# lxjeffffff/PagedAttention-Based-Transformer-Decoder-Inference-Framework

Hardware: AMD Instinct MI355X
Metric: decode tokens/sec at batch=64 seq_len=8192; % HBM-roofline (1/2/4/8 GPU) (higher is better)
Workload: dtype int8 GEMM (i32 acc) + fp16 KV attention (fp32 acc); 1 GPU; C3: INT8 decoder (MFMA i8 matmuls + fp16 paged attention), 24-layer/16-head/d=128, batch 64, KV context 8192, page 16; strong scaling: 64 rows over 1 GPU(s); global_batch=64, batch_per_gpu=64, seq_len=8192, page_size=16, parallelism=single GPU (no collective)

## Files before the change

### pagedattention-based-transformer-decoder-inference-framework_amd/csrc/gemm_impl.hpp

```cpp
#pragma once

#include "common.hpp"
#include "fp8.hpp"
#include "gemm.hpp"
#include "ln_wave.hpp"

namespace llm {

struct KvAppend {
  const int32_t* pos;
  const int32_t* page_table;
  const int32_t* rows;
  _Float16* k_pool;
  _Float16* v_pool;
  int num_beams, max_tiles, TS, num_pages, H, D;
  size_t page_stride;
  int fp8;
  float k_inv, v_inv;
};

struct GemmArgs {
  const uint8_t* A;
  int lda;
  int a_packed;
  const uint8_t* B;
  int M, N, K, KS;
  const float* sa;
  const float* sw;
  const float* bias;
  int act;
  float* C;
  int32_t* acc_out;
  int c_cols;
  int c_ld;
  _Float16* c16;
  KvAppend kv;
  unsigned long long* stamps;
  const float* ln_x;
  const _Float16* ln_emb;
  const int32_t* ln_tok;
  int ln_V;
  const float* ln_g;
  const float* ln_b;
  float ln_eps;
  uint8_t* act_out;
  float* sa_out;
  int partial;
  int w_keep;
  int xcd_map;
  unsigned* seam;
  int seam_n;
  int qdiag;
  int ksplit2;
};

__host__ __device__ constexpr int ln_row_stride(int K, int esize) { return K * esize + 32; }

__device__ __forceinline__ unsigned long long phase_clock() {
  unsigned long long t;
  asm volatile("s_memrealtime %0\n\ts_waitcnt lgkmcnt(0)" : "=s"(t)::"memory");
  return t;
}


template <int MT, int WAVES, int NT = 1>
constexpr int gemm_unroll() {
  return (MT >= 4 ? 2 : 4) * (WAVES == 4 ? 2 : 1) / (NT >= 4 ? 2 : 1);
}

__device__ __forceinline__ float apply_act(float y, int act) {
  if (act == LLM_ACT_RELU) return fmaxf(y, 0.f);
  if (act == LLM_ACT_GELU) return 0.5f * y * (1.f + erff(y * 0.70710678118654752f));
  return y;
}

enum class GemmKind { I8, F16 };

template <GemmKind KIND>
struct GemmTraits;
template <>
struct GemmTraits<GemmKind::I8> {
  static constexpr int KSTEP = 64, ESIZE = 1;
  using acc_t = i32x4;
  using elem_t = int32_t;
};
template <>
struct GemmTraits<GemmKind::F16> {
  static constexpr int KSTEP = 32, ESIZE = 2;
  using acc_t = f32x4;
  using elem_t = float;
};

template <GemmKind KIND, int ROWS, int WAVES>
__device__ __forceinline__ void ln_prologue(const GemmArgs& a, int m0, uint8_t* alds,
                                            float* sa_lds) {
  constexpr int ESIZE = GemmTraits<KIND>::ESIZE;
  constexpr int CPL = 8;
  const int lane = lane_id();
  const int w = wave_id_uniform();
  const int K = a.K;
  const int K4 = K >> 2;
  const int stride = ln_row_stride(K, ESIZE);
  const bool do_ln = a.ln_g != nullptr;
  LnRow<CPL> gm, bt;
  ln_wave_load(a.ln_g, K4, do_ln, gm);
  ln_wave_load(a.ln_b, K4, do_ln, bt);
  for (int r0 = w; r0 < ROWS; r0 += 2 * WAVES) {
    LnRow<CPL> x[2];
#pragma unroll
    for (int q = 0; q < 2; ++q) {
      const int r = r0 + q * WAVES;
      const int m = m0 + r;
      const bool ok = r < ROWS && m < a.M;
      if (a.ln_emb)
        ln_wave_load_f16(ok ? ln_embed_row(a.ln_emb, a.ln_tok, m, a.ln_V, K) : a.ln_emb, K4, ok,
                         x[q]);
      else
        ln_wave_load(a.ln_x + (size_t)m * K, K4, ok, x[q]);
    }
#pragma unroll
    for (int q = 0; q < 2; ++q) {
      const int r = r0 + q * WAVES;
      if (r >= ROWS) break;
      const bool mok = m0 + r < a.M;
      float am;
      if (do_ln) {
        am = ln_wave_compute(x[q], gm, bt, K, a.ln_eps);
      } else {
        am = 0.f;
#pragma unroll
        for (int j = 0; j < CPL; ++j)
#pragma unroll
          for (int e = 0; e < 4; ++e) am = fmaxf(am, fabsf(x[q].v[j][e]));
        am = ln_wave_max(am);
      }
      uint8_t* rowp = alds + (size_t)r * stride;
      if constexpr (KIND == GemmKind::I8) {
        const float scale = 127.f / (am + 1e-6f);
#pragma unroll
        for (int j = 0; j < CPL; ++j) {
          const int c = 64 * j + lane;
          if (c < K4)
            *reinterpret_cast<uint32_t*>(rowp + 4 * c) = mok ? ln_quant4(x[q].v[j], scale) : 0u;
        }
        if (lane == 0) sa_lds[r] = mok ? 1.0f / scale : 0.f;
      } else {
#pragma unroll
        for (int j = 0; j < CPL; ++j) {
          const int c = 64 * j + lane;
          if (c < K4)
            *reinterpret_cast<ln_f16x4*>(rowp + 8 * c) =
                mok ? ln_half4(x[q].v[j]) : ln_f16x4{0, 0, 0, 0};
        }
      }
    }
  }
}

__device__ __forceinline__ void seam_wait(unsigned* ctr, int n) {
  if (threadIdx.x == 0) {
    unsigned spins = 0;
    while (__hip_atomic_load(&ctr[0], __ATOMIC_RELAXED, __HIP_MEMORY_SCOPE_AGENT) < (unsigned)n) {
      __builtin_amdgcn_s_sleep(8);
      if (++spins > (1u << 21)) {
        __hip_atomic_store(&ctr[2], 1u, __ATOMIC_RELAXED, __HIP_MEMORY_SCOPE_AGENT);
        break;
      }
    }
    __builtin_amdgcn_fence(__ATOMIC_ACQUIRE, "agent");
  }
  __syncthreads();
}

template <GemmKind KIND, int MT, int NT, int WAVES, int DIAG = 0, int PRO = 0, int SEAM = 0>
__device__ __forceinline__ void gemm_tile(const GemmArgs& a, int bx, int by, int bz, int nz,
                                          int gx) {
  using Tr = GemmTraits<KIND>;
  using acc_t = typename Tr::acc_t;
  constexpr int KSTEP = Tr::KSTEP;
  constexpr int kUnroll = gemm_unroll<MT, WAVES, NT>();
  using elem_t = typename Tr::elem_t;
  using RedT = elem_t[MT * NT][4][64];
  extern __shared__ __attribute__((aligned(16))) uint8_t gemm_smem[];
  RedT* red;
  if constexpr (PRO == 0) {
    __shared__ elem_t red_static[WAVES][MT * NT][4][64];
    red = red_static;
  } else {
    red = reinterpret_cast<RedT*>(gemm_smem);
  }
  constexpr int ROWS_ = 16 * MT;
  const int a_stride = ln_row_stride(a.K, Tr::ESIZE);
  uint8_t* alds = gemm_smem;
  float* sa_lds = reinterpret_cast<float*>(gemm_smem + (size_t)ROWS_ * a_stride);

  const int lane = lane_id();
  const int w = wave_id_uniform();
  const int nt0 = bx * NT;
  const int m0 = by * 16 * MT;
  unsigned long long* stamp =
      a.stamps ? a.stamps + ((size_t)by * gx + bx) * 48 : nullptr;
  if (stamp && lane == 0) stamp[w] = phase_clock();
  const int wr = (w + bx) % WAVES;
  const int kz0 = (int)((bz * a.KS) / nz);
  const int kzn = (int)(((bz + 1) * a.KS) / nz) - kz0;
  const int ks0 = kz0 + (wr * kzn) / WAVES;
  const int ks1 = kz0 + ((wr + 1) * kzn) / WAVES;
  const int ntiles = (a.N + 15) >> 4;

  const int arow_lane = lane & 15;
  const int kgrp = lane >> 4;
  const bool apk = a.a_packed;
  const uint32_t a_bytes = apk ? (uint32_t)(((a.M + 15) / 16) * a.KS * 1024u)
                               : (uint32_t)((size_t)a.M * a.lda * Tr::ESIZE);
  const auto arsrc = __builtin_amdgcn_make_buffer_rsrc((void*)a.A, (short)0, a_bytes, 0x00020000);
  const uint32_t a_kstride = apk ? 1024u : (uint32_t)(KSTEP * Tr::ESIZE);
  const uint32_t a_kgrp_off = apk ? 0u : (uint32_t)(kgrp * (KSTEP / 4) * Tr::ESIZE);
  uint32_t a_row_off[MT];
#pragma unroll
  for (int mt = 0; mt < MT; ++mt) {
    const int row = m0 + mt * 16 + arow_lane;
    a_row_off[mt] = row >= a.M ? 0xFFFFFFF0u
                    : apk ? (uint32_t)((((m0 >> 4) + mt) * a.KS) * 1024u + lane * 16)
                          : (uint32_t)((size_t)row * a.lda * Tr::ESIZE);
  }
  const uint8_t* bbase = a.B + (size_t)nt0 * a.KS * 1024;
  const uint32_t b_bytes = (uint32_t)(min(NT, ntiles - nt0) * a.KS * 1024u);
  uint32_t b_lane_off[NT];
#pragma unroll
  for (int j = 0; j < NT; ++j) b_lane_off[j] = (uint32_t)j * a.KS * 1024u + lane * 16;
  const auto brsrc = __builtin_amdgcn_make_buffer_rsrc((void*)bbase, (short)0, b_bytes, 0x00020000);

  acc_t acc[MT][NT];
#pragma unroll
  for (int mt = 0; mt < MT; ++mt)
#pragma unroll
    for (int j = 0; j < NT; ++j) acc[mt][j] = acc_t{0, 0, 0, 0};

  struct Batch {
    u32x4 b[kUnroll][NT];
    u32x4 af[kUnroll][MT];
  };
  auto issue = [&](Batch& bt, int ks, bool do_a = true, bool do_b = true) {
#pragma unroll
    for (int u = 0; u < kUnroll; ++u) {
      const int kk = ks + u;
      const bool ok = kk < ks1;
#pragma unroll
      for (int j = 0; j < NT; ++j) {
        if (!do_b) break;
        const uint32_t boff = ok ? b_lane_off[j] + (uint32_t)kk * 1024u : 0xFFFFFFF0u;
        bt.b[u][j] = a.w_keep ? __builtin_amdgcn_raw_buffer_load_b128(brsrc, boff, 0, 0)
                              : __builtin_amdgcn_raw_buffer_load_b128(brsrc, boff, 0, 2);
      }
#pragma unroll
      for (int mt = 0; mt < MT; ++mt) {
        if (!do_a) break;
        if constexpr (PRO != 0) {
          const int r = mt * 16 + arow_lane;
          bt.af[u][mt] = ok ? *reinterpret_cast<const u32x4*>(alds + (size_t)r * a_stride +
                                                             16 * (4 * kk + kgrp))
                            : u32x4{0u, 0u, 0u, 0u};
          continue;
        }
        const uint32_t koff = (uint32_t)kk * a_kstride + a_kgrp_off;
        const uint32_t aoff = (ok && a_row_off[mt] != 0xFFFFFFF0u) ? a_row_off[mt] + koff : 0xFFFFFFF0u;
        if constexpr ((DIAG & 1) != 0)
          bt.af[u][mt] = u32x4{aoff, 0u, 0u, 0u};
        else
          bt.af[u][mt] = __builtin_amdgcn_raw_buffer_load_b128(arsrc, aoff, 0, 0);
      }
    }
  };
  auto compute = [&](const Batch& bt) {
#pragma unroll
    for (int u = 0; u < kUnroll; ++u) {
#pragma unroll
      for (int mt = 0; mt < MT; ++mt) {
        if constexpr (KIND == GemmKind::I8) {
#pragma unroll
          for (int j = 0; j < NT; ++j)
            acc[mt][j] = __builtin_amdgcn_mfma_i32_16x16x64_i8(
                __builtin_bit_cast(i32x4, bt.af[u][mt]), __builtin_bit_cast(i32x4, bt.b[u][j]),
                acc[mt][j], 0, 0, 0);
        } else if constexpr (KIND == GemmKind::F16) {
#pragma unroll
          for (int j = 0; j < NT; ++j)
            acc[mt][j] = __builtin_amdgcn_mfma_f32_16x16x32_f16(
                __builtin_bit_cast(f16x8, bt.af[u][mt]), __builtin_bit_cast(f16x8, bt.b[u][j]),
                acc[mt][j], 0, 0, 0);
        }
      }
    }
  };

  constexpr int ROWS = 16 * MT, COLS = 16 * NT, NTHR = WAVES * 64;
  constexpr int EPT = (ROWS * COLS + NTHR - 1) / NTHR;
  const KvAppend& kv = a.kv;
  const int hid = kv.H * kv.D;
  float e_scale[EPT], e_bias[EPT];
  int e_pos[EPT], e_br[EPT], e_page[EPT];
#pragma unroll
  for (int e = 0; e < EPT; ++e) {
    const int o = threadIdx.x + e * NTHR;
    const int m = m0 + o / COLS;
    const int n = nt0 * 16 + o % COLS;
    const bool valid = o < ROWS * COLS && m < a.M && n < a.N;
    e_scale[e] = 1.f;
    if constexpr (KIND == GemmKind::I8) {
      if (!PRO && valid && a.sa) e_scale[e] *= a.sa[m];
      if (valid && a.sw) e_scale[e] *= a.sw[n];
    }
    e_bias[e] = valid && a.bias && (!a.ksplit2 || bz == 0) ? a.bias[n] : 0.f;
    const bool kvcol = valid && kv.k_pool && n >= hid;
    e_pos[e] = kvcol ? kv.pos[m] : -1;
    e_br[e] = kvcol ? (kv.rows ? kv.rows[m] : m) : -1;
  }

  Batch b0, b1;
  bool b1_pre = false;
  if constexpr (PRO != 0) {
    bool pre = true;
#if LLM_TUNING
    pre = (a.qdiag & 2) == 0;
#endif
    if (pre && ks0 < ks1) issue(b0, ks0, false, true);
    if (pre && ks0 + kUnroll < ks1) {
      issue(b1, ks0 + kUnroll, false, true);
      b1_pre = true;
    }
    if constexpr (SEAM != 0) seam_wait(a.seam, a.seam_n);
#if LLM_TUNING
    if ((a.qdiag & 1) == 0)
#endif
    ln_prologue<KIND, ROWS_, WAVES>(a, m0, alds, sa_lds);
    __syncthreads();
    if constexpr (KIND == GemmKind::I8) {
#pragma unroll
      for (int e = 0; e < EPT; ++e) {
        const int o = threadIdx.x + e * NTHR;
        if (o < ROWS * COLS) e_scale[e] *= sa_lds[o / COLS];
      }
    }
    if (a.act_out && bx == 0) {
      const int KS = a.KS;
      for (int i = threadIdx.x; i < ROWS_ * KS * 4; i += NTHR) {
        const int r = i / (KS * 4), g = i % (KS * 4);
        const int m = m0 + r;
        if (m >= a.M) continue;
        const size_t off = ((size_t)((m >> 4) * KS + (g >> 2)) * 64 + (m & 15) + 16 * (g & 3)) * 16;
        *reinterpret_cast<u32x4*>(a.act_out + off) =
            *reinterpret_cast<const u32x4*>(alds + (size_t)r * a_stride + 16 * g);
      }
      if (KIND == GemmKind::I8 && a.sa_out && threadIdx.x < ROWS_ && m0 + (int)threadIdx.x < a.M)
        a.sa_out[m0 + threadIdx.x] = sa_lds[threadIdx.x];
    }
  }

  {
    int ks = ks0;
    bool b0_b = PRO == 0;
#if LLM_TUNING
    if constexpr (PRO != 0) b0_b = (a.qdiag & 2) != 0;
#endif
    if (ks < ks1) issue(b0, ks, true, b0_b);
#pragma unroll
    for (int e = 0; e < EPT; ++e) {
      const int o = threadIdx.x + e * NTHR;
      const int n = nt0 * 16 + o % COLS;
      const int p = e_pos[e], br = e_br[e];
      int page = -1;
      if (p >= 0 && br >= 0 && br < kv.num_beams && p / kv.TS < kv.max_tiles) {
        const int which = n >= 2 * hid;
        const int h = (n - hid * (1 + which)) / kv.D;
        page = kv.page_table[((size_t)br * kv.H + h) * kv.max_tiles + p / kv.TS];
        if (page >= kv.num_pages) page = -1;
      }
      e_page[e] = page;
    }
    while (ks < ks1) {
      if (ks + kUnroll < ks1) {
        issue(b1, ks + kUnroll, true, !b1_pre);
        b1_pre = false;
      }
      compute(b0);
      ks += kUnroll;
      if (ks >= ks1) break;
      if (ks + kUnroll < ks1) issue(b0, ks + kUnroll);
      compute(b1);
      ks += kUnroll;
    }
  }

  if (stamp && lane == 0) stamp[16 + w] = phase_clock();
  if constexpr ((DIAG & 2) != 0) {
    int32_t x = 0;
#pragma unroll
    for (int mt = 0; mt < MT; ++mt)
#pragma unroll
      for (int j = 0; j < NT; ++j) x ^= (int32_t)acc[mt][j][0] ^ (int32_t)acc[mt][j][3];
    if (lane == 0 && a.C) a.C[bx] = (float)x;
    if (stamp && lane == 0) stamp[32 + w] = phase_clock();
    return;
  }
  if constexpr (PRO != 0) __syncthreads();
#pragma unroll
  for (int mt = 0; mt < MT; ++mt)
#pragma unroll
    for (int j = 0; j < NT; ++j)
#pragma unroll
      for (int r = 0; r < 4; ++r) red[wr][mt * NT + j][r][lane] = acc[mt][j][r];
  __syncthreads();

#pragma unroll
  for (int e = 0; e < EPT; ++e) {
#pragma clang fp contract(off)
    const int o = threadIdx.x + e * NTHR;
    if (o >= ROWS * COLS) break;
    const int cl = o % COLS;
    const int row = o / COLS;
    const int j = cl >> 4;
    const int col = cl & 15;
    const int mt = row >> 4;
    const int rl = row & 15;
    const int src_lane = (rl >> 2) * 16 + col;
    const int reg = rl & 3;
    const int m = m0 + row;
    const int n = (nt0 + j) * 16 + col;
    if (m >= a.M || n >= a.N) continue;
    float y;
    if constexpr (KIND == GemmKind::I8) {
      int32_t s = 0;
#pragma unroll
      for (int ww = 0; ww < WAVES; ++ww) s += red[ww][mt * NT + j][reg][src_lane];
#if LLM_TUNING
      if (a.partial) {
        a.acc_out[((size_t)bz * a.M + m) * a.N + n] = s;
        continue;
      }
#endif
      if (a.acc_out) a.acc_out[(size_t)m * a.N + n] = s;
      y = (float)s * e_scale[e];
      if (a.bias) y = y + e_bias[e];
      if (a.ksplit2) {
        atomicAdd(a.C + (size_t)m * a.c_ld + n, y);
        continue;
      }
    } else {
      float s = 0.f;
#pragma unroll
      for (int ww = 0; ww < WAVES; ++ww) s += red[ww][mt * NT + j][reg][src_lane];
      y = a.bias ? s + e_bias[e] : s;
    }
    y = apply_act(y, a.act);
    if (a.C && n < a.c_cols) a.C[(size_t)m * a.c_ld + n] = y;
    if (a.c16) a.c16[a_frag_off_f16(m, n, a.N >> 5)] = (_Float16)y;
    if (e_page[e] >= 0) {
      const int which = n >= 2 * hid;
      const int i = n - hid * (1 + which);
      const int d = i % kv.D;
      const int p = e_pos[e];
      const size_t off = (size_t)e_page[e] * kv.page_stride + (size_t)(p % kv.TS) * kv.D + d;
      if (kv.fp8)
        reinterpret_cast<uint8_t*>(which ? kv.v_pool : kv.k_pool)[off] =
            (uint8_t)fp8_e4m3_byte(y, which ? kv.v_inv : kv.k_inv);
      else
        (which ? kv.v_pool : kv.k_pool)[off] = (_Float16)y;
    }
  }
  if (stamp && lane == 0) stamp[32 + w] = phase_clock();
}

template <GemmKind KIND, int MT, int NT, int WAVES, int DIAG = 0, int PRO = 0>
__global__ __launch_bounds__(WAVES * 64) void gemm_kernel(GemmArgs a) {
  int bx = blockIdx.x, by = blockIdx.y, bz = blockIdx.z;
#if LLM_TUNING
  if (a.xcd_map) {
    const int per = 8 / (int)gridDim.z;
    const int lin = blockIdx.x + gridDim.x * (blockIdx.y + gridDim.y * blockIdx.z);
    const int xcd = lin & 7;
    const int tile = (lin >> 3) * per + xcd % per;
    bz = xcd / per;
    bx = tile % (int)gridDim.x;
    by = tile / (int)gridDim.x;
  }
#endif
  gemm_tile<KIND, MT, NT, WAVES, DIAG, PRO>(a, bx, by, bz, (int)gridDim.z, (int)gridDim.x);
}

template <typename T, int EPL>
__global__ void pack_kernel(const T* __restrict__ W, T* __restrict__ P, int K, int N, int KS,
                            int ntiles) {
  const size_t idx = (size_t)blockIdx.x * blockDim.x + threadIdx.x;
  const size_t total = (size_t)ntiles * KS * 64;
  if (idx >= total) return;
  const int lane = idx & 63;
  const size_t blk = idx >> 6;
  const int ks = blk % KS;
  const int nt = blk / KS;
  const int n = nt * 16 + (lane & 15);
  const int kb = ks * (4 * EPL) + (lane >> 4) * EPL;
  T* dst = P + idx * EPL;
#pragma unroll
  for (int j = 0; j < EPL; ++j) {
    const int k = kb + j;
    dst[j] = (k < K && n < N) ? W[(size_t)k * N + n] : T(0);
  }
}

namespace {

inline int pick_nt(int N, int M) {
  if (M <= 16) return 1;
  const int ntiles = (N + 15) / 16;
  const int mblocks = (M + 63) / 64;
  return (ntiles % 2 == 0 && (ntiles / 2) * mblocks >= 192) ? 2 : 1;
}

template <GemmKind KIND, int MT, int NT, int WAVES>
size_t ln_lds_bytes(int K) {
  const size_t img = (size_t)16 * MT * ln_row_stride(K, GemmTraits<KIND>::ESIZE) + 16 * MT * 4;
  const size_t red = (size_t)WAVES * MT * NT * 4 * 64 * 4;
  return img > red ? img : red;
}
constexpr size_t kLnLdsMax = 160 * 1024;

template <GemmKind KIND, int MT, int NT>
hipError_t launch_gemm_nt(const GemmArgs& a, int waves, int mblocks, hipStream_t st, int kslices) {
  const int ntiles = (a.N + 15) / 16;
  const dim3 grid((ntiles + NT - 1) / NT, mblocks, kslices);
  if constexpr (NT <= 2) {
    if (a.ln_x) {
      const size_t lds = ln_lds_bytes<KIND, MT, NT, 8>(a.K);
      hipLaunchKernelGGL((gemm_kernel<KIND, MT, NT, 8, 0, 1>), grid, dim3(512), lds, st, a);
      return hipGetLastError();
    }
  }
  if constexpr (MT * NT * 8 <= 64) {
    if (waves != 4) {
      hipLaunchKernelGGL((gemm_kernel<KIND, MT, NT, 8>), grid, dim3(512), 0, st, a);
      return hipGetLastError();
    }
  }
  hipLaunchKernelGGL((gemm_kernel<KIND, MT, NT, 4>), grid, dim3(256), 0, st, a);
  return hipGetLastError();
}

template <GemmKind KIND, int MT>
hipError_t launch_gemm_mt(const GemmArgs& a, int NT, int waves, int mblocks, hipStream_t st,
                          int kslices) {
#if LLM_TUNING
  if (NT == 4 && !a.ln_x) return launch_gemm_nt<KIND, MT, 4>(a, waves, mblocks, st, kslices);
  if (NT == 3 && !a.ln_x) return launch_gemm_nt<KIND, MT, 3>(a, waves, mblocks, st, kslices);
#endif
  return NT == 2 ? launch_gemm_nt<KIND, MT, 2>(a, waves, mblocks, st, kslices)
                 : launch_gemm_nt<KIND, MT, 1>(a, waves, mblocks, st, kslices);
}

}

namespace {

inline int pick_waves(const GemmArgs&, int) { return 8; }

struct TileChoice {
  int nt, waves, mrows;
};
inline bool narrow_tile_for(int M, int N, int K, TileChoice& t) {
  if (M <= 16 || M > 64) return false;
  const int ntiles = (N + 15) / 16;
  if (M > 32) {
    if (ntiles >= 256) return false;
    t = TileChoice{2, 8, 16};
    return true;
  }
  if (ntiles < 384) {
    t = K >= 4096 ? TileChoice{1, 8, 16} : TileChoice{1, 4, 16};
    return true;
  }
  if (ntiles < 512) {
    t = TileChoice{1, 4, 16};
    return true;
  }
  return false;
}
inline bool narrow_decode_tile(const GemmArgs& a, int kstep, TileChoice& t) {
  if ((a.ln_x && a.ln_g) || a.partial) return false;
  if (a.ksplit2 && a.M > 32 && a.M <= 64) {
    t = TileChoice{2, 8, 64};
    return true;
  }
  return narrow_tile_for(a.M, a.N, a.KS * kstep, t);
}

template <GemmKind KIND>
hipError_t launch_gemm(const GemmArgs& a_in, hipStream_t st, int nt_override = 0,
                       int waves_override = 0, int mrows_override = 0, int ks_override = 0) {
  GemmArgs a = a_in;
  TileChoice tc{0, 0, 0};
  const bool narrow = nt_override == 0 && waves_override == 0 && mrows_override == 0 &&
                      narrow_decode_tile(a, GemmTraits<KIND>::KSTEP, tc);
  if (narrow) {
    nt_override = tc.nt;
    waves_override = tc.waves;
    mrows_override = tc.mrows;
  }
  const int NT = nt_override > 0 ? nt_override : pick_nt(a.N, a.M);
  const int waves = waves_override > 0 ? waves_override : pick_waves(a, NT);
  int mrows = a.M <= 16 ? 16 : a.M <= 32 ? 32 : 64;
  if (mrows == 64 && NT == 1 && (a.N + 15) / 16 < 256 && !a.ln_x && !a.partial) mrows = 32;
  if (mrows_override > 0) mrows = mrows_override;
  const int ks = a.partial ? std::max(1, ks_override) : a.ksplit2 ? 2 : 1;
  const int mblocks = (a.M + mrows - 1) / mrows;
  const int tiles = ((a.N + 15) / 16 + NT - 1) / NT * mblocks;
  if (a.xcd_map && (ks < 2 || 8 % ks != 0 || (tiles * ks) % 8 != 0)) a.xcd_map = 0;
  if (mrows == 16) return launch_gemm_mt<KIND, 1>(a, NT, waves, mblocks, st, ks);
  if (mrows == 32) return launch_gemm_mt<KIND, 2>(a, NT, waves, mblocks, st, ks);
  return launch_gemm_mt<KIND, 4>(a, NT, waves, mblocks, st, ks);
}

}
}
```

### pagedattention-based-transformer-decoder-inference-framework_amd/csrc/tune/gemm_tune.hip

```cpp
#include "gemm_impl.hpp"

using namespace llm;

__global__ void gemm_end_stamp_kernel(unsigned long long* t) {
  if (threadIdx.x == 0) *t = phase_clock();
}

extern "C" int i8_gemm_stamps(int nt, int waves, int mrows, const int8_t* A, const void* W_packed,
                              float* C, int M, int N, int K, const float* sa, const float* sw,
                              unsigned long long* stamps, unsigned long long* end_stamp,
                              void* stream) {
  GemmArgs a{};
  a.a_packed = 1;
  a.A = reinterpret_cast<const uint8_t*>(A);
  a.lda = K;
  a.B = static_cast<const uint8_t*>(W_packed);
  a.M = M; a.N = N; a.K = K; a.KS = K / 64;
  a.sa = sa; a.sw = sw; a.C = C; a.c_cols = N; a.c_ld = N;
  a.stamps = stamps;
  hipStream_t st = as_stream(stream);
  hipError_t e = hipSuccess;
  const int ntiles = N / 16;
  const int diag = waves >> 8;
  if (diag == 0) {
    e = launch_gemm<GemmKind::I8>(a, st, nt, waves, mrows);
  } else {
    LLM_REQUIRE((nt == 2 && mrows == 64) || (nt == 1 && mrows == 32), "i8_gemm_stamps: diag shape");
    auto go = [&](auto kern, int NTv, int mr) {
      hipLaunchKernelGGL(kern, dim3((ntiles + NTv - 1) / NTv, (M + mr - 1) / mr), dim3(512), 0, st, a);
    };
    if (nt == 2) {
      if (diag == 1) go(gemm_kernel<GemmKind::I8, 4, 2, 8, 1>, 2, 64);
      else if (diag == 2) go(gemm_kernel<GemmKind::I8, 4, 2, 8, 2>, 2, 64);
      else go(gemm_kernel<GemmKind::I8, 4, 2, 8, 3>, 2, 64);
    } else {
      if (diag == 1) go(gemm_kernel<GemmKind::I8, 2, 1, 8, 1>, 1, 32);
      else if (diag == 2) go(gemm_kernel<GemmKind::I8, 2, 1, 8, 2>, 1, 32);
      else go(gemm_kernel<GemmKind::I8, 2, 1, 8, 3>, 1, 32);
    }
    e = hipGetLastError();
  }
  if (e == hipSuccess) {
    hipLaunchKernelGGL(gemm_end_stamp_kernel, dim3(1), dim3(64), 0, st, end_stamp);
    e = hipGetLastError();
  }
  return e == hipSuccess ? LLM_OK : fail(LLM_ERR_HIP, "i8_gemm_stamps");
}

extern "C" int i8_gemm_tune(int nt, int waves, int mrows, int a_packed, const int8_t* A, int lda,
                            const void* W_packed, float* C, int M, int N, int K, const float* sa,
                            const float* sw, void* stream) {
  GemmArgs a{};
  a.a_packed = a_packed;
  a.A = reinterpret_cast<const uint8_t*>(A);
  a.lda = lda;
  a.B = static_cast<const uint8_t*>(W_packed);
  a.M = M; a.N = N; a.K = K; a.KS = K / 64;
  a.sa = sa; a.sw = sw; a.C = C; a.c_cols = N; a.c_ld = N;
  hipError_t e = launch_gemm<GemmKind::I8>(a, as_stream(stream), nt, waves, mrows);
  return e == hipSuccess ? LLM_OK : fail(LLM_ERR_HIP, "i8_gemm_tune");
}

extern "C" int i8_gemm_tune_qpro(const float* x, const void* W_packed, float* C, int M, int N,
                                 int K, const float* sw, int qdiag, void* stream) {
  LLM_REQUIRE(quant_prologue_ok(M, N, K), "i8_gemm_tune_qpro: shape");
  GemmArgs a{};
  a.a_packed = 1;
  a.B = static_cast<const uint8_t*>(W_packed);
  a.M = M; a.N = N; a.K = K; a.KS = K / 64;
  a.sw = sw; a.C = C; a.c_cols = N; a.c_ld = N;
  a.ln_x = x;
  a.ln_eps = 1e-5f;
  a.qdiag = qdiag;
  hipError_t e = launch_gemm<GemmKind::I8>(a, as_stream(stream));
  return e == hipSuccess ? LLM_OK : fail(LLM_ERR_HIP, "i8_gemm_tune_qpro");
}

extern "C" int i8_gemm_tune_sk(int nt, int waves, int mrows, int kslices, int xcd_map,
                               const int8_t* A, const void* W_packed, int32_t* acc_out, int M,
                               int N, int K, void* stream) {
  LLM_REQUIRE(kslices >= 1 && kslices <= 8 && K % 64 == 0 && N % 16 == 0, "i8_gemm_tune_sk: shape");
  GemmArgs a{};
  a.a_packed = 1;
  a.A = reinterpret_cast<const uint8_t*>(A);
  a.lda = K;
  a.B = static_cast<const uint8_t*>(W_packed);
  a.M = M; a.N = N; a.K = K; a.KS = K / 64;
  a.partial = 1;
  a.acc_out = acc_out;
  a.xcd_map = xcd_map;
  hipError_t e = launch_gemm<GemmKind::I8>(a, as_stream(stream), nt, waves, mrows, kslices);
  return e == hipSuccess ? LLM_OK : fail(LLM_ERR_HIP, "i8_gemm_tune_sk");
}

__global__ __launch_bounds__(512) void gemm_pair_f16_kernel(GemmArgs a1, GemmArgs a2, int n1,
                                                            unsigned* sync) {
  const int wg = blockIdx.x;
  if (wg < n1) {
    gemm_tile<GemmKind::F16, 1, 1, 8, 0, 0>(a1, wg, 0, 0, 1, n1);
    __syncthreads();
    if (threadIdx.x == 0) {
      __builtin_amdgcn_fence(__ATOMIC_RELEASE, "agent");
      __hip_atomic_fetch_add(&sync[0], 1u, __ATOMIC_RELAXED, __HIP_MEMORY_SCOPE_AGENT);
    }
  }
  gemm_tile<GemmKind::F16, 1, 1, 8, 0, 1, 1>(a2, wg, 0, 0, 1, (int)gridDim.x);
  if (threadIdx.x == 0) {
    const unsigned old = __hip_atomic_fetch_add(&sync[1], 1u, __ATOMIC_RELAXED, __HIP_MEMORY_SCOPE_AGENT);
    if (old == gridDim.x - 1) {
      __hip_atomic_store(&sync[0], 0u, __ATOMIC_RELAXED, __HIP_MEMORY_SCOPE_AGENT);
      __hip_atomic_store(&sync[1], 0u, __ATOMIC_RELAXED, __HIP_MEMORY_SCOPE_AGENT);
    }
  }
}

extern "C" int f16_gemm_pair_tune(const void* A1, const void* W1, float* x, const float* ln_g,
                                  const float* ln_b, const void* W2, const float* b2, void* C16,
                                  int M, int K, int N1, int N2, unsigned* sync, int fused,
                                  void* stream) {
  LLM_REQUIRE(M >= 1 && M <= 16 && K == N1 && K % 32 == 0 && N1 % 16 == 0 && N2 % 32 == 0 &&
                  ln_fusable(LLM_F16, M, K) && N2 / 16 >= N1 / 16 && N2 / 16 <= 256,
              "f16_gemm_pair_tune: shape");
  GemmArgs a1{};
  a1.a_packed = 1;
  a1.A = static_cast<const uint8_t*>(A1);
  a1.B = static_cast<const uint8_t*>(W1);
  a1.M = M; a1.N = N1; a1.K = K; a1.KS = K / 32;
  a1.C = x; a1.c_cols = N1; a1.c_ld = N1;
  a1.w_keep = 1;
  GemmArgs a2{};
  a2.a_packed = 1;
  a2.B = static_cast<const uint8_t*>(W2);
  a2.M = M; a2.N = N2; a2.K = N1; a2.KS = N1 / 32;
  a2.bias = b2; a2.act = LLM_ACT_RELU;
  a2.c16 = static_cast<_Float16*>(C16);
  a2.c_cols = 0; a2.c_ld = N2;
  a2.ln_x = x; a2.ln_g = ln_g; a2.ln_b = ln_b; a2.ln_eps = 1e-5f;
  a2.w_keep = 1;
  a2.seam = sync;
  a2.seam_n = N1 / 16;
  hipStream_t st = as_stream(stream);
  hipError_t e;
  if (!fused) {
    e = launch_gemm<GemmKind::F16>(a1, st);
    if (e == hipSuccess) e = launch_gemm<GemmKind::F16>(a2, st);
  } else {
    const size_t lds = ln_lds_bytes<GemmKind::F16, 1, 1, 8>(N1);
    hipLaunchKernelGGL(gemm_pair_f16_kernel, dim3(N2 / 16), dim3(512), lds, st, a1, a2, N1 / 16,
                       sync);
    e = hipGetLastError();
  }
  return e == hipSuccess ? LLM_OK : fail(LLM_ERR_HIP, "f16_gemm_pair_tune");
}

extern "C" int f16_gemm_tune(int nt, int waves, int mrows, int a_packed, const void* A, int lda,
                             const void* W_packed, float* C, int M, int N, int K, void* stream) {
  GemmArgs a{};
  a.a_packed = a_packed;
  a.A = static_cast<const uint8_t*>(A);
  a.lda = lda;
  a.B = static_cast<const uint8_t*>(W_packed);
  a.M = M; a.N = N; a.K = K; a.KS = K / 32;
  a.C = C; a.c_cols = N; a.c_ld = N;
  hipError_t e = launch_gemm<GemmKind::F16>(a, as_stream(stream), nt, waves, mrows);
  return e == hipSuccess ? LLM_OK : fail(LLM_ERR_HIP, "f16_gemm_tune");
}
```

Baseline: 3797 tokens/s.

## Stage packed int8 activations into LDS via global_load_lds for MT=4 GEMMs

Adds a PRO=2 GEMM form. For each 64-row block, the block's packed int8 activation tile is copied once into LDS with global_load_lds, together with the first weight prefetches, and the MFMA loop then reads A from LDS instead of issuing buffer loads from global memory on every k-step. It is enabled by default for int8 GEMMs with MT=4, NT<=2, 8 waves, no k-split and M<=64, which matches batch 64. Diagnostic variants for load ordering and late epilogue operand loads are added for tuning. In exchange it needs up to 160KB of dynamic LDS, which can limit occupancy, and it adds a full vmcnt(0) wait before compute.

```diff
diff --git a/pagedattention-based-transformer-decoder-inference-framework_amd/csrc/gemm_impl.hpp b/pagedattention-based-transformer-decoder-inference-framework_amd/csrc/gemm_impl.hpp
--- a/pagedattention-based-transformer-decoder-inference-framework_amd/csrc/gemm_impl.hpp
+++ b/pagedattention-based-transformer-decoder-inference-framework_amd/csrc/gemm_impl.hpp
@@ -51,6 +51,7 @@
   unsigned* seam;
   int seam_n;
   int qdiag;
+  int lds_a;
   int ksplit2;
 };
 
@@ -183,6 +184,7 @@
   using RedT = elem_t[MT * NT][4][64];
   extern __shared__ __attribute__((aligned(16))) uint8_t gemm_smem[];
   RedT* red;
+  static_assert(PRO != 2 || (KIND == GemmKind::I8 && SEAM == 0), "LDS-A form: packed int8 A");
   if constexpr (PRO == 0) {
     __shared__ elem_t red_static[WAVES][MT * NT][4][64];
     red = red_static;
@@ -241,11 +243,9 @@
     u32x4 b[kUnroll][NT];
     u32x4 af[kUnroll][MT];
   };
+  constexpr bool a_first = (DIAG & 4) != 0;
   auto issue = [&](Batch& bt, int ks, bool do_a = true, bool do_b = true) {
-#pragma unroll
-    for (int u = 0; u < kUnroll; ++u) {
-      const int kk = ks + u;
-      const bool ok = kk < ks1;
+    auto issue_b = [&](int u, int kk, bool ok) {
 #pragma unroll
       for (int j = 0; j < NT; ++j) {
         if (!do_b) break;
@@ -253,10 +253,23 @@
         bt.b[u][j] = a.w_keep ? __builtin_amdgcn_raw_buffer_load_b128(brsrc, boff, 0, 0)
                               : __builtin_amdgcn_raw_buffer_load_b128(brsrc, boff, 0, 2);
       }
+    };
+#pragma unroll
+    for (int u = 0; u < kUnroll; ++u) {
+      const int kk = ks + u;
+      const bool ok = kk < ks1;
+      if constexpr (!a_first) issue_b(u, kk, ok);
 #pragma unroll
       for (int mt = 0; mt < MT; ++mt) {
         if (!do_a) break;
-        if constexpr (PRO != 0) {
+        if constexpr (PRO == 2 && (DIAG & 1) == 0) {
+          bt.af[u][mt] = (ok && m0 + 16 * mt < a.M)
+                             ? *reinterpret_cast<const u32x4*>(
+                                   alds + ((size_t)(mt * a.KS + kk) * 1024 + lane * 16))
+                             : u32x4{0u, 0u, 0u, 0u};
+          continue;
+        }
+        if constexpr (PRO == 1) {
           const int r = mt * 16 + arow_lane;
           bt.af[u][mt] = ok ? *reinterpret_cast<const u32x4*>(alds + (size_t)r * a_stride +
                                                              16 * (4 * kk + kgrp))
@@ -270,6 +283,7 @@
         else
           bt.af[u][mt] = __builtin_amdgcn_raw_buffer_load_b128(arsrc, aoff, 0, 0);
       }
+      if constexpr (a_first) issue_b(u, kk, ok);
     }
   };
   auto compute = [&](const Batch& bt) {
@@ -300,26 +314,56 @@
   const int hid = kv.H * kv.D;
   float e_scale[EPT], e_bias[EPT];
   int e_pos[EPT], e_br[EPT], e_page[EPT];
-#pragma unroll
-  for (int e = 0; e < EPT; ++e) {
-    const int o = threadIdx.x + e * NTHR;
-    const int m = m0 + o / COLS;
-    const int n = nt0 * 16 + o % COLS;
-    const bool valid = o < ROWS * COLS && m < a.M && n < a.N;
-    e_scale[e] = 1.f;
-    if constexpr (KIND == GemmKind::I8) {
-      if (!PRO && valid && a.sa) e_scale[e] *= a.sa[m];
-      if (valid && a.sw) e_scale[e] *= a.sw[n];
-    }
-    e_bias[e] = valid && a.bias && (!a.ksplit2 || bz == 0) ? a.bias[n] : 0.f;
-    const bool kvcol = valid && kv.k_pool && n >= hid;
-    e_pos[e] = kvcol ? kv.pos[m] : -1;
-    e_br[e] = kvcol ? (kv.rows ? kv.rows[m] : m) : -1;
-  }
+  constexpr bool epi_late = (DIAG & 8) != 0;
+  auto load_epilogue_operands = [&]() {
+#pragma unroll
+    for (int e = 0; e < EPT; ++e) {
+      const int o = threadIdx.x + e * NTHR;
+      const int m = m0 + o / COLS;
+      const int n = nt0 * 16 + o % COLS;
+      const bool valid = o < ROWS * COLS && m < a.M && n < a.N;
+      e_scale[e] = 1.f;
+      if constexpr (KIND == GemmKind::I8) {
+        if (PRO != 1 && valid && a.sa) e_scale[e] *= a.sa[m];
+        if (valid && a.sw) e_scale[e] *= a.sw[n];
+      }
+      e_bias[e] = valid && a.bias && (!a.ksplit2 || bz == 0) ? a.bias[n] : 0.f;
+      const bool kvcol = valid && kv.k_pool && n >= hid;
+      e_pos[e] = kvcol ? kv.pos[m] : -1;
+      e_br[e] = kvcol ? (kv.rows ? kv.rows[m] : m) : -1;
+    }
+  };
+  if constexpr (!epi_late) load_epilogue_operands();
 
   Batch b0, b1;
   bool b1_pre = false;
-  if constexpr (PRO != 0) {
+  if constexpr (PRO == 2) {
+    constexpr bool copy_first = (DIAG & 16) == 0;
+    auto pre_weights = [&]() {
+      if (ks0 < ks1) issue(b0, ks0, false, true);
+      if (ks0 + kUnroll < ks1) {
+        issue(b1, ks0 + kUnroll, false, true);
+        b1_pre = true;
+      }
+    };
+    if constexpr (!copy_first) pre_weights();
+    if constexpr ((DIAG & 1) == 0) {
+#pragma unroll
+      for (int mt = 0; mt < MT; ++mt) {
+        if (m0 + 16 * mt >= a.M) break;
+        const uint8_t* src = a.A + ((size_t)((m0 >> 4) + mt) * a.KS) * 1024 + lane * 16;
+        for (int kk = ks0; kk < ks1; ++kk)
+          __builtin_amdgcn_global_load_lds(
+              (const __attribute__((address_space(1))) void*)(src + (size_t)kk * 1024),
+              (__attribute__((address_space(3))) void*)(alds + (size_t)(mt * a.KS + kk) * 1024),
+              16, 0, 0);
+      }
+    }
+    if constexpr (copy_first) pre_weights();
+    if constexpr (epi_late) load_epilogue_operands();
+    asm volatile("s_waitcnt vmcnt(0)" ::: "memory");
+  }
+  if constexpr (PRO == 1) {
     bool pre = true;
 #if LLM_TUNING
     pre = (a.qdiag & 2) == 0;
@@ -361,9 +405,10 @@
     int ks = ks0;
     bool b0_b = PRO == 0;
 #if LLM_TUNING
-    if constexpr (PRO != 0) b0_b = (a.qdiag & 2) != 0;
+    if constexpr (PRO == 1) b0_b = (a.qdiag & 2) != 0;
 #endif
     if (ks < ks1) issue(b0, ks, true, b0_b);
+    if constexpr (epi_late && PRO != 2) load_epilogue_operands();
 #pragma unroll
     for (int e = 0; e < EPT; ++e) {
       const int o = threadIdx.x + e * NTHR;
@@ -526,9 +571,49 @@
 constexpr size_t kLnLdsMax = 160 * 1024;
 
 template <GemmKind KIND, int MT, int NT>
+bool lds_a_ok(const GemmArgs& a, int waves, int kslices) {
+  if (KIND != GemmKind::I8 || NT > 2 || waves == 4 || kslices != 1) return false;
+  if (!a.a_packed || a.ln_x || a.partial || a.ksplit2) return false;
+  return (size_t)16 * MT * a.K <= kLnLdsMax;
+}
+template <int MT, int NT>
+bool lds_a_ships(const GemmArgs& a) {
+  return MT == 4 && a.M <= 64;
+}
+#if LLM_TUNING
+constexpr bool kLdsAEveryForm = true;
+#else
+constexpr bool kLdsAEveryForm = false;
+#endif
+template <int MT, int NT>
+size_t lds_a_bytes(int K) {
+  const size_t img = (size_t)16 * MT * K;
+  const size_t red = (size_t)8 * MT * NT * 4 * 64 * 4;
+  return img > red ? img : red;
+}
+
+template <GemmKind KIND, int MT, int NT>
 hipError_t launch_gemm_nt(const GemmArgs& a, int waves, int mblocks, hipStream_t st, int kslices) {
   const int ntiles = (a.N + 15) / 16;
   const dim3 grid((ntiles + NT - 1) / NT, mblocks, kslices);
+  if constexpr (KIND == GemmKind::I8 && NT <= 2 && (MT == 4 || kLdsAEveryForm)) {
+    bool lds_a = lds_a_ok<KIND, MT, NT>(a, waves, kslices) && lds_a_ships<MT, NT>(a);
+#if LLM_TUNING
+    if (a.lds_a != 0) lds_a = a.lds_a > 0 && lds_a_ok<KIND, MT, NT>(a, waves, kslices);
+#endif
+    if (lds_a) {
+      const size_t lds = lds_a_bytes<MT, NT>(a.K);
+      const auto kern = gemm_kernel<KIND, MT, NT, 8, 0, 2>;
+      static bool attr = false;
+      if (!attr) {
+        (void)hipFuncSetAttribute(reinterpret_cast<const void*>(kern),
+                                  hipFuncAttributeMaxDynamicSharedMemorySize, (int)kLnLdsMax);
+        attr = true;
+      }
+      hipLaunchKernelGGL(kern, grid, dim3(512), lds, st, a);
+      return hipGetLastError();
+    }
+  }
   if constexpr (NT <= 2) {
     if (a.ln_x) {
       const size_t lds = ln_lds_bytes<KIND, MT, NT, 8>(a.K);
diff --git a/pagedattention-based-transformer-decoder-inference-framework_amd/csrc/tune/gemm_tune.hip b/pagedattention-based-transformer-decoder-inference-framework_amd/csrc/tune/gemm_tune.hip
--- a/pagedattention-based-transformer-decoder-inference-framework_amd/csrc/tune/gemm_tune.hip
+++ b/pagedattention-based-transformer-decoder-inference-framework_amd/csrc/tune/gemm_tune.hip
@@ -4,6 +4,48 @@
 
 __global__ void gemm_end_stamp_kernel(unsigned long long* t) {
   if (threadIdx.x == 0) *t = phase_clock();
+}
+
+namespace {
+
+template <int MT, int NT, int DIAG, int PRO>
+void launch_diag(const GemmArgs& a, hipStream_t st) {
+  const dim3 grid(((a.N + 15) / 16 + NT - 1) / NT, (a.M + 16 * MT - 1) / (16 * MT));
+  const auto kern = gemm_kernel<GemmKind::I8, MT, NT, 8, DIAG, PRO>;
+  size_t lds = 0;
+  if (PRO == 2) {
+    lds = lds_a_bytes<MT, NT>(a.K);
+    (void)hipFuncSetAttribute(reinterpret_cast<const void*>(kern),
+                              hipFuncAttributeMaxDynamicSharedMemorySize, (int)kLnLdsMax);
+  }
+  hipLaunchKernelGGL(kern, grid, dim3(512), lds, st, a);
+}
+
+template <int MT, int NT>
+bool launch_diag_form(const GemmArgs& a, int diag, int lds_a, hipStream_t st) {
+  if (lds_a) {
+    if (!lds_a_ok<GemmKind::I8, MT, NT>(a, 8, 1)) return false;
+    switch (diag) {
+      case 0: launch_diag<MT, NT, 0, 2>(a, st); return true;
+      case 1: launch_diag<MT, NT, 1, 2>(a, st); return true;
+      case 2: launch_diag<MT, NT, 2, 2>(a, st); return true;
+      case 3: launch_diag<MT, NT, 3, 2>(a, st); return true;
+      case 8: launch_diag<MT, NT, 8, 2>(a, st); return true;
+      case 16: launch_diag<MT, NT, 16, 2>(a, st); return true;
+      default: return false;
+    }
+  }
+  switch (diag) {
+    case 1: launch_diag<MT, NT, 1, 0>(a, st); return true;
+    case 2: launch_diag<MT, NT, 2, 0>(a, st); return true;
+    case 3: launch_diag<MT, NT, 3, 0>(a, st); return true;
+    case 4: launch_diag<MT, NT, 4, 0>(a, st); return true;
+    case 8: launch_diag<MT, NT, 8, 0>(a, st); return true;
+    case 12: launch_diag<MT, NT, 12, 0>(a, st); return true;
+    default: return false;
+  }
+}
+
 }
 
 extern "C" int i8_gemm_stamps(int nt, int waves, int mrows, const int8_t* A, const void* W_packed,
@@ -20,24 +62,25 @@
   a.stamps = stamps;
   hipStream_t st = as_stream(stream);
   hipError_t e = hipSuccess;
-  const int ntiles = N / 16;
-  const int diag = waves >> 8;
-  if (diag == 0) {
+  const int diag = (waves >> 8) & 0xff;
+  const int lds_a = (waves >> 16) & 1;
+  waves &= 0xff;
+  LLM_REQUIRE(waves == 8 && (nt == 1 || nt == 2) && (mrows == 16 || mrows == 32 || mrows == 64),
+              "i8_gemm_stamps: 8 waves, 1 or 2 column tiles, 16 / 32 / 64 rows");
+  if (diag == 0 && !lds_a) {
+    a.lds_a = -1;
     e = launch_gemm<GemmKind::I8>(a, st, nt, waves, mrows);
   } else {
-    LLM_REQUIRE((nt == 2 && mrows == 64) || (nt == 1 && mrows == 32), "i8_gemm_stamps: diag shape");
-    auto go = [&](auto kern, int NTv, int mr) {
-      hipLaunchKernelGGL(kern, dim3((ntiles + NTv - 1) / NTv, (M + mr - 1) / mr), dim3(512), 0, st, a);
-    };
-    if (nt == 2) {
-      if (diag == 1) go(gemm_kernel<GemmKind::I8, 4, 2, 8, 1>, 2, 64);
-      else if (diag == 2) go(gemm_kernel<GemmKind::I8, 4, 2, 8, 2>, 2, 64);
-      else go(gemm_kernel<GemmKind::I8, 4, 2, 8, 3>, 2, 64);
-    } else {
-      if (diag == 1) go(gemm_kernel<GemmKind::I8, 2, 1, 8, 1>, 1, 32);
-      else if (diag == 2) go(gemm_kernel<GemmKind::I8, 2, 1, 8, 2>, 1, 32);
-      else go(gemm_kernel<GemmKind::I8, 2, 1, 8, 3>, 1, 32);
-    }
+    bool ok;
+    if (nt == 2)
+      ok = mrows == 64   ? launch_diag_form<4, 2>(a, diag, lds_a, st)
+           : mrows == 32 ? launch_diag_form<2, 2>(a, diag, lds_a, st)
+                         : launch_diag_form<1, 2>(a, diag, lds_a, st);
+    else
+      ok = mrows == 64   ? launch_diag_form<4, 1>(a, diag, lds_a, st)
+           : mrows == 32 ? launch_diag_form<2, 1>(a, diag, lds_a, st)
+                         : launch_diag_form<1, 1>(a, diag, lds_a, st);
+    LLM_REQUIRE(ok, "i8_gemm_stamps: diag value, or a shape the LDS-A form does not take");
     e = hipGetLastError();
   }
   if (e == hipSuccess) {
@@ -59,6 +102,34 @@
   a.sa = sa; a.sw = sw; a.C = C; a.c_cols = N; a.c_ld = N;
   hipError_t e = launch_gemm<GemmKind::I8>(a, as_stream(stream), nt, waves, mrows);
   return e == hipSuccess ? LLM_OK : fail(LLM_ERR_HIP, "i8_gemm_tune");
+}
+
+extern "C" int i8_gemm_tune_lds(int lds_a, int nt, int waves, int mrows, int a_packed,
+                                const int8_t* A, int lda, const void* W_packed, int32_t* acc_out,
+                                float* C, int M, int N, int K, const float* sa, const float* sw,
+                                const float* bias, int act, void* stream) {
+  GemmArgs a{};
+  a.a_packed = a_packed;
+  a.A = reinterpret_cast<const uint8_t*>(A);
+  a.lda = lda;
+  a.B = static_cast<const uint8_t*>(W_packed);
+  a.M = M; a.N = N; a.K = K; a.KS = K / 64;
+  a.sa = sa; a.sw = sw; a.bias = bias; a.act = act;
+  a.C = C; a.acc_out = acc_out; a.c_cols = N; a.c_ld = N;
+  a.lds_a = lds_a;
+  hipError_t e = launch_gemm<GemmKind::I8>(a, as_stream(stream), nt, waves, mrows);
+  return e == hipSuccess ? LLM_OK : fail(LLM_ERR_HIP, "i8_gemm_tune_lds");
+}
+
+extern "C" int i8_gemm_lds_a_form(int nt, int mrows, int a_packed, int K) {
+  GemmArgs a{};
+  a.a_packed = a_packed;
+  a.K = K;
+  if (nt < 1 || nt > 2) return 0;
+  return mrows == 64   ? lds_a_ok<GemmKind::I8, 4, 2>(a, 8, 1)
+         : mrows == 32 ? lds_a_ok<GemmKind::I8, 2, 2>(a, 8, 1)
+         : mrows == 16 ? lds_a_ok<GemmKind::I8, 1, 2>(a, 8, 1)
+                       : 0;
 }
 
 extern "C" int i8_gemm_tune_qpro(const float* x, const void* W_packed, float* C, int M, int N,
```

Result: no change. 3804 tokens/s (median of 6 runs) (+0.2%).
